# whoiszzj/APD-MVS

Measured on AMD Instinct MI355X. Metric: Mpix*iterations/sec (PatchMatch sweep), higher is better.
Workload: dtype f32

## Files before the change

apd-mvs_amd/csrc/apd_kernels_k67w.hip:

```cpp
#include "apd_device.h"
#include "apd_sweep.h"
#include "apd_window.h"


namespace apd {

constexpr int kWinH = APD_WIN_H;

template <bool kQuad>
__device__ __forceinline__ SrcWindow stage_window(const FrameArgs &fa, const ViewConst &vc, uint32_t *win, bool alive, int px, int py,
                                                  const float4 plane, bool trusted, bool enabled)
{
    if (!enabled) {
        SrcWindow none;
        none.valid = 0;
        none.wx0 = none.wy0 = none.addr0 = 0;
        none.lo_x = none.lo_y = 3.0e38f;
        none.hi_x = none.hi_y = -3.0e38f;
        return none;
    }
    float cx = 0.0f, cy = 0.0f;
    bool ok = false;
    if (alive) {
        float qx, qy, qz;
        plane_q(plane, qx, qy, qz);
        const Homography H = make_homography(fa, vc, qx, qy, qz);
        correspond(H, (float)px, (float)py, cx, cy);
        ok = cx >= 0.0f && cx < vc.wf && cy >= 0.0f && cy < vc.hf;
    }
    if (__builtin_amdgcn_ballot_w64(ok && trusted) != 0) {
        ok = ok && trusted;
    }
    return stage_window_around<kQuad, kWinH>(fa, vc, win, ok, cx, cy);
}

constexpr float kTrustedCost = 0.5f;
constexpr int kWinFromIter = 1;

template <int NMAX, bool kQuad, bool kTiled, bool kApprox>
__global__ __launch_bounds__(256, kQuad ? APD_K67W_WAVES : APD_K67W_WAVES_F32) void k67w_update_strong(FrameArgs fa, int colour, int iter)
{
    __shared__ float tile[kLdsH * kLdsPitch];
    __shared__ uint32_t windows[4][window_dwords(kWinH)];
    __shared__ uint16_t refine_items[4][5 * 64];
    __shared__ float refine_cost[4][5][64];
    const TilePixel t = checkerboard_pixel(fa, colour);
    for (int idx = threadIdx.x; idx < kLdsW * kLdsH; idx += 256) {
        const int r = idx / kLdsW, c = idx - r * kLdsW;
        tile[r * kLdsPitch + c] = fetch_texel(fa.ref_img, fa.W, fa.H, t.tx0 + c - kHalo, t.ty0 + r - kHalo);
    }
    __syncthreads();
    uint32_t *win = windows[threadIdx.x >> 6];
    const int px = t.px, py = t.py;
    const int center = py * fa.W + px;
    const bool alive = checkerboard_active(fa, t) && fa.weak_info[center] != APD_WEAK && !masked_out(fa, center);
    if (__builtin_amdgcn_ballot_w64(alive) == 0) {
        return;
    }
    const RefPatchLds<kLdsPitch> rp = ref_patch_from_lds<kLdsPitch>(&tile[t.ly * kLdsPitch + t.lx]);

    const int nsrc = fa.num_src;
    Rng rng = Rng{0, 0, 0, 0, 0, 0};
    float cost_array[9][NMAX];
    int positions[8];
    unsigned flags = 0;
    ViewWeights<NMAX> vw;
    vw.clear();
    float weight_norm = 0.0f;
    uint32_t sel = 0;
    float4 plane_now = make_float4(0.0f, 0.0f, 1.0f, 1.0f);
    float depth_now = 0.0f, cost_now = 0.0f, cost_committed = 0.0f;
    float ref_w[5];
    float4 ref_normals[5];
    float tc[5] = {0.0f, 0.0f, 0.0f, 0.0f, 0.0f};

    const bool use_windows = !(fa.state == APD_FIRST_INIT && iter < kWinFromIter);
    bool trusted = false;
    if (alive) {
        plane_now = fa.planes[center];
        trusted = fa.costs[center] < kTrustedCost;
#pragma unroll 1
        for (int h = 0; h < 8; ++h) {
            int pos = 0;
            if (arm_candidate(fa, px, py, h, pos)) {
                flags |= 1u << h;
            }
            positions[h] = pos;
        }
    }

#pragma unroll 1
    for (int v = 0; v < nsrc; ++v) {
        const ViewConst &vc = view_const(fa, v);
        const SrcWindow w = stage_window<kQuad>(fa, vc, win, alive, px, py, plane_now, trusted, use_windows);
        if (alive) {
#pragma unroll 1
            for (int h = 0; h < 9; ++h) {
                if (h < 8 && !(flags & (1u << h))) {
                    cost_array[h][v] = (h == 0 && v == 0) ? 2.0f : 0.0f;
                    continue;
                }
                const float4 pl = (h < 8) ? fa.planes[positions[h]] : plane_now;
                float qx, qy, qz;
                plane_q(pl, qx, qy, qz);
                cost_array[h][v] = ncc_fixed_windowed<kQuad, kWinW, kTiled, kApprox>(fa, vc, w, rp, px, py, qx, qy, qz);
            }
        }
    }

    if (alive) {
        float priors[NMAX];
        for (int j = 0; j < NMAX; ++j) {
            priors[j] = 0.0f;
        }
        const int nb_pos[4] = {center - fa.W, center + fa.W, center - 1, center + 1};
        for (int i = 0; i < 4; ++i) {
            if (flags & (1u << (2 * i))) {
                const uint32_t sv = fa.selected_views[nb_pos[i]];
                for (int j = 0; j < nsrc; ++j) {
                    priors[j] += bit_test(sv, (unsigned)j) == 1 ? 0.9f : 0.1f;
                }
            }
        }
        rng = rng_load(fa.rng, center);
        select_views<NMAX>(fa, iter, cost_array, priors, rng, vw, sel, weight_norm);
        vw.store(fa, center);
        float final_costs[8];
        for (int i = 0; i < 8; ++i) {
            float f = 0.0f;
            for (int j = 0; j < nsrc; ++j) {
                const uint32_t wj = vw.get(j);
                if (wj > 0) {
                    f += (float)wj * cost_array[i][j];
                }
            }
            final_costs[i] = f / weight_norm;
        }
        int best = 0;
        float best_c = final_costs[0];
        for (int i = 1; i < 8; ++i) {
            if (final_costs[i] <= best_c) {
                best_c = final_costs[i];
                best = i;
            }
        }
        cost_now = 0.0f;
        for (int i = 0; i < nsrc; ++i) {
            cost_now += (float)vw.get(i) * cost_array[8][i];
        }
        cost_now /= weight_norm;
        cost_committed = cost_now;
        depth_now = depth_from_plane(fa, plane_now, px, py);
        if (flags & (1u << best)) {
            const float4 cand = fa.planes[positions[best]];
            const float d = depth_from_plane(fa, cand, px, py);
            if (d >= fa.depth_min && d <= fa.depth_max && final_costs[best] < cost_now) {
                depth_now = d;
                plane_now = cand;
                cost_now = final_costs[best];
                fa.selected_views[center] = sel;
            }
        }
        float ref_depths[5];
        trusted = cost_now < kTrustedCost;
        make_refinement_set(fa, px, py, rng, plane_now, depth_now, ref_depths, ref_normals);
        rng_store(fa.rng, center, rng);
#pragma unroll
        for (int k = 0; k < 5; ++k) {
            ref_w[k] = distance_to_origin(fa, px, py, ref_depths[k], ref_normals[k].x, ref_normals[k].y, ref_normals[k].z);
        }
    }

    const float lost = refinement_lost_bound(fa, cost_now, weight_norm);
    const int lane = threadIdx.x & 63, wave_id = threadIdx.x >> 6;
    uint16_t *items = refine_items[wave_id];
    float(*costs_out)[64] = refine_cost[wave_id];
    const int wave_lx0 = (wave_id % kWavesX) * kWaveW, wave_ly0 = (wave_id / kWavesX) * kWaveH;
#pragma unroll 1
    for (int v = 0; v < nsrc; ++v) {
        const uint32_t wv = alive ? vw.get(v) : 0u;
        unsigned open = 0;
        if (wv > 0) {
#pragma unroll
            for (int k = 0; k < 5; ++k) {
                open |= (tc[k] >= lost) ? 0u : (1u << k);
            }
        }
        constexpr int kOrder[5] = {1, 3, 4, 0, 2};
        int off[6];
        off[0] = 0;
#pragma unroll
        for (int j = 0; j < 5; ++j) {
            const int k = kOrder[j];
            const unsigned long long m = __builtin_amdgcn_ballot_w64((open >> k) & 1u);
            if ((open >> k) & 1u) {
                const int rank = (int)__builtin_amdgcn_mbcnt_hi((unsigned)(m >> 32), __builtin_amdgcn_mbcnt_lo((unsigned)m, 0u));
                items[off[j] + rank] = (uint16_t)((k << 6) | lane);
            }
            off[j + 1] = off[j] + __builtin_popcountll(m);
        }
        const int total = off[5];
        if (total == 0) {
            continue;
        }
        __builtin_amdgcn_fence(__ATOMIC_RELEASE, "wavefront");
        __builtin_amdgcn_wave_barrier();
        const ViewConst &vc = view_const(fa, v);
        const SrcWindow w = stage_window<kQuad>(fa, vc, win, alive, px, py, plane_now, trusted, use_windows);
#pragma unroll 1
        for (int first = 0; first < total; first += 64) {
            const int idx = first + lane;
            const bool valid = idx < total;
            const unsigned item = valid ? (unsigned)items[idx] : 0u;
            const int owner = (int)(item & 63u), hyp = (int)(item >> 6);
            const int last = min(total, first + 64) - 1;
            int j_lo = 0, j_hi = 0;
#pragma unroll
            for (int j = 1; j < 5; ++j) {
                j_lo += off[j] <= first ? 1 : 0;
                j_hi += off[j] <= last ? 1 : 0;
            }
            float4 pl = make_float4(0.0f, 0.0f, 1.0f, 1.0f);
#pragma unroll 1
            for (int j = j_lo; j <= j_hi; ++j) {
                const int k = (0x20431 >> (4 * j)) & 7;
                const float nx = __shfl(ref_normals[k].x, owner), ny = __shfl(ref_normals[k].y, owner), nz = __shfl(ref_normals[k].z, owner);
                const float nw = __shfl(ref_w[k], owner);
                if (hyp == k) {
                    pl = make_float4(nx, ny, nz, nw);
                }
            }
            RefPatchLds<kLdsPitch> orp;
            orp.mean = __shfl(rp.mean, owner);
            orp.var = __shfl(rp.var, owner);
            const int oly = wave_ly0 + owner / kWaveLanesX;
            const int olx = wave_lx0 + 2 * (owner % kWaveLanesX) + ((oly + colour) & 1);
            orp.base = &tile[oly * kLdsPitch + olx];
            if (valid) {
                float qx, qy, qz;
                plane_q(pl, qx, qy, qz);
                costs_out[hyp][owner] = ncc_fixed_windowed<kQuad, kWinW, kTiled, kApprox>(fa, vc, w, orp, t.tx0 + olx, t.ty0 + oly, qx, qy, qz);
            }
        }
        __builtin_amdgcn_fence(__ATOMIC_RELEASE, "wavefront");
        __builtin_amdgcn_wave_barrier();
#pragma unroll
        for (int k = 0; k < 5; ++k) {
            if ((open >> k) & 1u) {
                tc[k] += (float)wv * costs_out[k][lane];
            }
        }
        __builtin_amdgcn_fence(__ATOMIC_RELEASE, "wavefront");
        __builtin_amdgcn_wave_barrier();
    }

    if (!alive) {
        return;
    }
#pragma unroll 1
    for (int k = 0; k < 5; ++k) {
        float4 pl = ref_normals[k];
        pl.w = ref_w[k];
        const float c = tc[k] / weight_norm;
        const float d = depth_from_plane(fa, pl, px, py);
        if (d >= fa.depth_min && d <= fa.depth_max && c < cost_now) {
            depth_now = d;
            plane_now = pl;
            cost_now = c;
        }
    }
    if (fa.state == APD_REFINE_INIT) {
        if ((double)cost_now < (double)cost_committed - 0.1) {
            fa.costs[center] = cost_now;
            fa.planes[center] = plane_now;
        } else {
            fa.costs[center] = cost_committed;
        }
    } else {
        fa.costs[center] = cost_now;
        fa.planes[center] = plane_now;
    }
}


template <bool kQuad, bool kTiled, bool kApprox>
static void launch_k67w_n(const FrameArgs &fa, int tiles, int colour, int iter, hipStream_t s)
{
    with_view_capacity(fa.num_src, [&](auto nmax) {
        hipLaunchKernelGGL((k67w_update_strong<decltype(nmax)::value, kQuad, kTiled, kApprox>), dim3(tiles), dim3(256), 0, s, fa, colour, iter);
    });
}

template <bool kQuad, bool kTiled>
static void launch_k67w(const FrameArgs &fa, int tiles, int colour, int iter, hipStream_t s)
{
    if (fa.approx_rcp) {
        launch_k67w_n<kQuad, kTiled, true>(fa, tiles, colour, iter, s);
    } else {
        launch_k67w_n<kQuad, kTiled, false>(fa, tiles, colour, iter, s);
    }
}

hipError_t launch_k67_windowed(const FrameArgs &fa, int colour, int iter, hipStream_t s)
{
    const int tiles = ((fa.W + kTileW - 1) / kTileW) * ((fa.H + kTileH - 1) / kTileH);
    if (fa.use_quads) {
        const int mode = fa.tiled_mode;
        const bool windows_off = fa.state == APD_FIRST_INIT && iter < kWinFromIter;
        if (fa.have_tiled && (mode == 2 || (mode == 1 && windows_off))) {
            launch_k67w<true, true>(fa, tiles, colour, iter, s);
        } else {
            launch_k67w<true, false>(fa, tiles, colour, iter, s);
        }
    } else {
        launch_k67w<false, false>(fa, tiles, colour, iter, s);
    }
    return hipGetLastError();
}

}


APD_WIN_STATS_ACCESSOR(apd_debug_win_stats)
```

apd-mvs_amd/csrc/apd_tuning.h:

```cpp
#pragma once

#ifndef APD_ROW_PREFETCH
#define APD_ROW_PREFETCH 1
#endif

#ifndef APD_CB_ROWS
#define APD_CB_ROWS 4
#endif
#ifndef APD_FF_ROWS
#define APD_FF_ROWS 8
#endif

#ifndef APD_WIN_H
#define APD_WIN_H (kWaveH + 16)
#endif
#ifndef APD_K67W_WAVES
#define APD_K67W_WAVES 4
#endif
#ifndef APD_K67W_WAVES_F32
#define APD_K67W_WAVES_F32 3
#endif

#ifndef APD_FW_TILE_PITCH
#define APD_FW_TILE_PITCH (kFwLds + 1)
#endif
#ifndef APD_K1415_WIN_PITCH
#define APD_K1415_WIN_PITCH 72
#endif
#ifndef APD_K14_WIN_H
#define APD_K14_WIN_H 32
#endif
#ifndef APD_K14_PAIRS_FROM_N
#define APD_K14_PAIRS_FROM_N 10
#endif
#ifndef APD_K14_PAIRS_FROM_N_PHOTO
#define APD_K14_PAIRS_FROM_N_PHOTO 8
#endif
#ifndef APD_K14_PAIRS_FROM_N_GEOM
#define APD_K14_PAIRS_FROM_N_GEOM 2
#endif
#ifndef APD_K14_PAIRS_MIN_SAVE
#define APD_K14_PAIRS_MIN_SAVE 2
#endif
#ifndef APD_K14_CHUNK
#define APD_K14_CHUNK 8
#endif
#ifndef APD_K14W_WAVES
#define APD_K14W_WAVES 4
#endif
#ifndef APD_K1415W_WAVES_F32
#define APD_K1415W_WAVES_F32 3
#endif

#ifndef APD_WEAK_SUPER_SHIFT
#define APD_WEAK_SUPER_SHIFT 4
#endif
#ifndef APD_K910_WIN_H
#define APD_K910_WIN_H 28
#endif
#ifndef APD_K910_WAVES
#define APD_K910_WAVES 2
#endif
```

apd-mvs_amd/csrc/apd_window.h:

```cpp
#pragma once

#include "apd_device.h"


namespace apd {

constexpr int kWinW = 64;
constexpr int window_dwords(int winh, int pitch = kWinW) { return pitch * (winh + 1); }
static_assert(kQuadShift == 2, "the window is staged from dword fetches of the quad image");

template <bool kQuad> struct WinEntry;
template <> struct WinEntry<true> {
    typedef uint32_t type;
};
template <> struct WinEntry<false> {
    typedef pair_t type;
};
constexpr int kWinEntryShift = 2;

typedef __attribute__((address_space(3))) uint32_t *lds_u32_ptr;

__device__ __forceinline__ int lds_address(uint32_t *p)
{
#if defined(__HIP_DEVICE_COMPILE__)
    return (int)(uintptr_t)(lds_u32_ptr)p;
#else
    return 0;
#endif
}

template <typename E>
struct WinTaps {
    E top, bot;
};

template <typename E, int kPitch>
__device__ __forceinline__ WinTaps<E> lds_read_pair(int addr)
{
    WinTaps<E> t;
#if defined(__HIP_DEVICE_COMPILE__)
    typedef __attribute__((address_space(3))) E *lds_ptr;
    const lds_ptr p = (lds_ptr)(uintptr_t)(uint32_t)addr;
    t.top = p[0];
    t.bot = p[kPitch];
#else
    t.top = t.bot = E();
#endif
    return t;
}

template <int kPitch>
__device__ __forceinline__ WinTaps<pair_t> lds_read_texels(int addr)
{
    WinTaps<pair_t> t;
#if defined(__HIP_DEVICE_COMPILE__)
    typedef __attribute__((address_space(3))) float *lds_ptr;
    const lds_ptr p = (lds_ptr)(uintptr_t)(uint32_t)addr;
    t.top.x = p[0];
    t.top.y = p[1];
    t.bot.x = p[kPitch];
    t.bot.y = p[kPitch + 1];
#else
    t.top = t.bot = pair_t();
#endif
    return t;
}


struct SrcWindow {
    int valid;
    int wx0, wy0;
    float lo_x, hi_x, lo_y, hi_y;
    int addr0;
};

__device__ __forceinline__ float wave_min(float v)
{
#pragma unroll
    for (int m = 32; m >= 1; m >>= 1) {
        v = fminf(v, __shfl_xor(v, m));
    }
    return v;
}

__device__ __forceinline__ float wave_max(float v)
{
#pragma unroll
    for (int m = 32; m >= 1; m >>= 1) {
        v = fmaxf(v, __shfl_xor(v, m));
    }
    return v;
}

template <bool kQuad, int WINH, int kPitch = kWinW>
__device__ __forceinline__ SrcWindow stage_window_around(const FrameArgs &fa, const ViewConst &vc, uint32_t *win, bool ok, float cx, float cy)
{
    constexpr int kWinRows = WINH + 1;
    SrcWindow w;
    const float big = 3.0e38f;
    const float x_lo = wave_min(ok ? cx : big), x_hi = wave_max(ok ? cx : -big);
    const float y_lo = wave_min(ok ? cy : big), y_hi = wave_max(ok ? cy : -big);
    if (!(x_lo <= x_hi)) {
        w.valid = 0;
        w.wx0 = w.wy0 = w.addr0 = 0;
        w.lo_x = w.lo_y = big;
        w.hi_x = w.hi_y = -big;
        return w;
    }
    const int wx0 = __builtin_amdgcn_readfirstlane((int)floorf(0.5f * (x_lo + x_hi)) - kWinW / 2);
    const int wy0 = __builtin_amdgcn_readfirstlane((int)floorf(0.5f * (y_lo + y_hi)) - WINH / 2);
    const int lane = threadIdx.x & 63;
    const int col = med3_i32(wx0 + lane, -1, fa.W - 1) + 1;
    if constexpr (kQuad) {
        const global_quad_ptr srcq = (global_quad_ptr)vc.quad;
        const unsigned rpitch = quad_row_pitch_bytes(fa.W);
        constexpr int kLoads = (kWinRows + 1) / 2;
        uint32_t tmp[kLoads];
#pragma unroll
        for (int k = 0; k < kLoads; ++k) {
            const int gy = min(max(wy0 + 2 * k, -1), fa.H - 1);
            tmp[k] = quad_fetch(srcq, (unsigned)(gy + 1) * rpitch + ((unsigned)col << kRowEntryShift));
        }
#pragma unroll
        for (int k = 0; k < kLoads; ++k) {
            float t0, t1, x0, x1;
            asm("v_cvt_f32_ubyte0 %0, %1" : "=v"(t0) : "v"(tmp[k]));
            asm("v_cvt_f32_ubyte1 %0, %1" : "=v"(t1) : "v"(tmp[k]));
            asm("v_cvt_f32_ubyte2 %0, %1" : "=v"(x0) : "v"(tmp[k]));
            asm("v_cvt_f32_ubyte3 %0, %1" : "=v"(x1) : "v"(tmp[k]));
            win[(2 * k) * kPitch + lane] = __builtin_bit_cast(uint32_t, __builtin_amdgcn_cvt_pkrtz(t0, x0 - t0));
            if (2 * k + 1 < kWinRows) {
                win[(2 * k + 1) * kPitch + lane] = __builtin_bit_cast(uint32_t, __builtin_amdgcn_cvt_pkrtz(t1, x1 - t1));
            }
        }
    } else {
        typedef const __attribute__((address_space(1))) float *global_float_ptr;
        const global_float_ptr img = (global_float_ptr)vc.img;
        float *winf = reinterpret_cast<float *>(win);
        const int cx = med3_i32(wx0 + lane, 0, fa.W - 1);
        float tmp[kWinRows];
#pragma unroll
        for (int k = 0; k < kWinRows; ++k) {
            const int gy = min(max(wy0 + k, 0), fa.H - 1);
            tmp[k] = img[(unsigned)(gy * fa.W + cx)];
        }
#pragma unroll
        for (int k = 0; k < kWinRows; ++k) {
            winf[k * kPitch + lane] = tmp[k];
        }
    }
    __builtin_amdgcn_fence(__ATOMIC_RELEASE, "wavefront");
    __builtin_amdgcn_wave_barrier();
    if ((threadIdx.x & 63) == 0) {
        APD_WIN_COUNT(5, 1);
    }
    w.valid = 1;
    w.wx0 = wx0;
    w.wy0 = wy0;
    w.lo_x = (float)max(wx0 + 1, 0);
    w.hi_x = (float)(wx0 + kWinW - (kQuad ? 1 : 2));
    w.lo_y = (float)max(wy0 + 1, 0);
    w.hi_y = (float)(wy0 + WINH - 1);
    w.addr0 = __builtin_amdgcn_readfirstlane(lds_address(win) - (wy0 * kPitch + wx0) * (1 << kWinEntryShift));
    return w;
}

template <int kShift, int kPitch>
__device__ __forceinline__ int win_byte_address(int qx, int qy, int addr0)
{
    int row, off;
    asm("v_mad_i32_i24 %0, %1, %2, %3" : "=v"(row) : "v"(qy), "v"(kPitch << kShift), "v"(addr0));
    asm("v_lshl_add_u32 %0, %1, %3, %2" : "=v"(off) : "v"(qx), "v"(row), "n"(kShift));
    return off;
}

template <bool kQuad, int kPitch, bool kApprox = false, bool kEnds = false>
__device__ __forceinline__ void win_row_issue(const Homography &H, float bx, float by, float bz, const float (&yf)[kPatchN], int addr0,
                                              float (&a)[kPatchN], float (&b)[kPatchN],
                                              WinTaps<typename WinEntry<kQuad>::type> (&t)[kPatchN], float Xa = 0.0f, float Ya = 0.0f,
                                              float Xb = 0.0f, float Yb = 0.0f)
{
    constexpr int j0 = kEnds ? 1 : 0, j1 = kEnds ? kPatchN - 1 : kPatchN;
    float z[kPatchN], X[kPatchN], Y[kPatchN], r[kPatchN];
#pragma unroll
    for (int j = j0; j < j1; ++j) {
        z[j] = fmaf(H.h[7], yf[j], bz);
        X[j] = fmaf(H.h[1], yf[j], bx);
        Y[j] = fmaf(H.h[4], yf[j], by);
    }
    APD_STAGE();
#pragma unroll
    for (int j = j0; j < j1; ++j) {
        r[j] = __builtin_amdgcn_rcpf(z[j]);
    }
    APD_STAGE();
    if constexpr (!kApprox) {
#pragma unroll
        for (int j = j0; j < j1; ++j) {
            z[j] = fmaf(-z[j], r[j], 1.0f);
        }
        APD_STAGE();
#pragma unroll
        for (int j = j0; j < j1; ++j) {
            r[j] = fmaf(z[j], r[j], r[j]);
        }
        APD_STAGE();
    }
#pragma unroll
    for (int j = j0; j < j1; ++j) {
        X[j] *= r[j];
        Y[j] *= r[j];
    }
    if constexpr (kEnds) {
        X[0] = Xa;
        Y[0] = Ya;
        X[kPatchN - 1] = Xb;
        Y[kPatchN - 1] = Yb;
    }
    APD_STAGE();
    constexpr float kEntryBytes = (float)(1 << kWinEntryShift), kPitchBytes = (float)(kPitch << kWinEntryShift);
    const float addr0f = (float)addr0 + 8388608.0f;
    float fx[kPatchN], fy[kPatchN];
#pragma unroll
    for (int j = 0; j < kPatchN; ++j) {
        a[j] = __builtin_amdgcn_fractf(X[j]);
        b[j] = __builtin_amdgcn_fractf(Y[j]);
    }
    APD_STAGE();
#pragma unroll
    for (int j = 0; j < kPatchN; ++j) {
        fx[j] = X[j] - a[j];
        fy[j] = Y[j] - b[j];
    }
    APD_STAGE();
#pragma unroll
    for (int j = 0; j < kPatchN; ++j) {
        fx[j] = fmaf(fx[j], kEntryBytes, addr0f);
    }
    APD_STAGE();
#pragma unroll
    for (int j = 0; j < kPatchN; ++j) {
        fx[j] = fmaf(fy[j], kPitchBytes, fx[j]);
    }
    APD_STAGE();
    int addr[kPatchN];
#pragma unroll
    for (int j = 0; j < kPatchN; ++j) {
        addr[j] = (int)(__float_as_uint(fx[j]) & 0x007FFFFFu);
    }
    APD_STAGE();
#pragma unroll
    for (int j = 0; j < kPatchN; ++j) {
        if constexpr (kQuad) {
            t[j] = lds_read_pair<uint32_t, kPitch>(addr[j]);
        } else {
            t[j] = lds_read_texels<kPitch>(addr[j]);
        }
    }
}

template <bool kQuad>
__device__ __forceinline__ void win_row_lerp(const WinTaps<typename WinEntry<kQuad>::type> (&t)[kPatchN], const float (&a)[kPatchN],
                                             const float (&b)[kPatchN], float (&v)[kPatchN])
{
    float top[kPatchN], bot[kPatchN];
#pragma unroll
    for (int j = 0; j < kPatchN; ++j) {
        if constexpr (kQuad) {
            top[j] = lerp_f16_pair(a[j], t[j].top);
            bot[j] = lerp_f16_pair(a[j], t[j].bot);
        } else {
            top[j] = fmaf(a[j], t[j].top.y - t[j].top.x, t[j].top.x);
            bot[j] = fmaf(a[j], t[j].bot.y - t[j].bot.x, t[j].bot.x);
        }
    }
    APD_STAGE();
#pragma unroll
    for (int j = 0; j < kPatchN; ++j) {
        bot[j] -= top[j];
    }
    APD_STAGE();
#pragma unroll
    for (int j = 0; j < kPatchN; ++j) {
        v[j] = fmaf(b[j], bot[j], top[j]);
    }
}

__device__ __forceinline__ float opaque_f32(float v)
{
    asm volatile("" : "+v"(v));
    return v;
}

template <bool kQuad, int kPitch, bool kApprox, bool kLocal = false, typename Ref>
__device__ __forceinline__ void ncc_window_moments(const Ref &rp, const Homography &H, int px, int py, int addr0, float &sum_s,
                                                   float &sum_ss, float &sum_rs, const float (&cX)[4], const float (&cY)[4])
{
    float yf[kPatchN];
    float x_first = 0.0f;
    if constexpr (kLocal) {
        x_first = opaque_f32((float)(px - kPatchRadius));
        const float y_first = opaque_f32((float)(py - kPatchRadius));
#pragma unroll
        for (int j = 0; j < kPatchN; ++j) {
            yf[j] = y_first + (float)(kPatchStep * j);
        }
    } else {
#pragma unroll
        for (int j = 0; j < kPatchN; ++j) {
            yf[j] = (float)(py + kPatchStep * j - kPatchRadius);
        }
    }
    sum_s = 0.0f;
    sum_ss = 0.0f;
    sum_rs = 0.0f;
    __builtin_amdgcn_s_setprio(1);
    __builtin_amdgcn_s_waitcnt(0xC07F);
    float a[2][kPatchN], b[2][kPatchN];
    WinTaps<typename WinEntry<kQuad>::type> t[2][kPatchN];
    {
        const float xf = kLocal ? x_first : (float)(px - kPatchRadius);
        win_row_issue<kQuad, kPitch, kApprox, true>(H, fmaf(H.h[0], xf, H.h[2]), fmaf(H.h[3], xf, H.h[5]), fmaf(H.h[6], xf, H.h[8]), yf,
                                                      addr0, a[0], b[0], t[0], cX[0], cY[0], cX[1], cY[1]);
    }
#pragma unroll
    for (int i = 0; i < kPatchN; ++i) {
        float v[kPatchN];
        float ref[kPatchN];
#pragma unroll
        for (int j = 0; j < kPatchN; ++j) {
            ref[j] = rp.at(i, j);
        }
        APD_STAGE();
        if (i + 2 < kPatchN) {
            const float xf = kLocal ? x_first + (float)(kPatchStep * (i + 1)) : (float)(px + kPatchStep * (i + 1) - kPatchRadius);
            win_row_issue<kQuad, kPitch, kApprox>(H, fmaf(H.h[0], xf, H.h[2]), fmaf(H.h[3], xf, H.h[5]), fmaf(H.h[6], xf, H.h[8]), yf,
                                                  addr0, a[(i + 1) & 1], b[(i + 1) & 1], t[(i + 1) & 1]);
        } else if (i + 1 < kPatchN) {
            const float xf = kLocal ? x_first + (float)(kPatchStep * (i + 1)) : (float)(px + kPatchStep * (i + 1) - kPatchRadius);
            win_row_issue<kQuad, kPitch, kApprox, true>(H, fmaf(H.h[0], xf, H.h[2]), fmaf(H.h[3], xf, H.h[5]), fmaf(H.h[6], xf, H.h[8]), yf,
                                                          addr0, a[(i + 1) & 1], b[(i + 1) & 1], t[(i + 1) & 1], cX[2], cY[2], cX[3], cY[3]);
        }
        APD_STAGE();
        win_row_lerp<kQuad>(t[i & 1], a[i & 1], b[i & 1], v);
        float row_s = 0.0f, row_ss = 0.0f, row_rs = 0.0f;
#pragma unroll
        for (int j = 0; j < kPatchN; ++j) {
            row_s += v[j];
            row_ss = fmaf(v[j], v[j], row_ss);
            row_rs = fmaf(ref[j], v[j], row_rs);
        }
        sum_s += row_s;
        sum_ss += row_ss;
        sum_rs += row_rs;
    }
    __builtin_amdgcn_s_setprio(0);
}

template <bool kApprox = false>
__device__ __forceinline__ void corner_position(const Homography &H, float xf, float yf, float &X, float &Y)
{
    const float z = fmaf(H.h[7], yf, fmaf(H.h[6], xf, H.h[8]));
    const float r = kApprox ? __builtin_amdgcn_rcpf(z) : recip_fast(z);
    X = fmaf(H.h[1], yf, fmaf(H.h[0], xf, H.h[2])) * r;
    Y = fmaf(H.h[4], yf, fmaf(H.h[3], xf, H.h[5])) * r;
}

template <bool kQuad, int kPitch = kWinW, bool kTiled = false, bool kApprox = false, bool kLocal = false, typename Ref>
__device__ __forceinline__ float ncc_fixed_windowed(const FrameArgs &fa, const ViewConst &vc, const SrcWindow &w, const Ref &rp, int px,
                                                    int py, float qx, float qy, float qz)
{
    const Homography H = make_homography(fa, vc, qx, qy, qz);
    float cx, cy;
    correspond(H, (float)px, (float)py, cx, cy);
    if (cx >= vc.wf || cx < 0.0f || cy >= vc.hf || cy < 0.0f) {
        return 2.0f;
    }
    const float kMinVar = 1e-5f;
    if (rp.var < kMinVar) {
        return 2.0f;
    }
    const float x0 = (float)(px - kPatchRadius), x1 = (float)(px + kPatchRadius);
    const float y0 = (float)(py - kPatchRadius), y1 = (float)(py + kPatchRadius);
    const bool fast_recip = denominators_fast(H, x0, x1, y0, y1);
    bool in_window = false;
    float cX[4], cY[4];
    if (fast_recip && w.valid) {
        corner_position<kApprox>(H, x0, y0, cX[0], cY[0]);
        corner_position<kApprox>(H, x0, y1, cX[1], cY[1]);
        corner_position<kApprox>(H, x1, y0, cX[2], cY[2]);
        corner_position<kApprox>(H, x1, y1, cX[3], cY[3]);
        const float xl = fminf(fminf(cX[0], cX[1]), fminf(cX[2], cX[3])), xh = fmaxf(fmaxf(cX[0], cX[1]), fmaxf(cX[2], cX[3]));
        const float yl = fminf(fminf(cY[0], cY[1]), fminf(cY[2], cY[3])), yh = fmaxf(fmaxf(cY[0], cY[1]), fmaxf(cY[2], cY[3]));
        in_window = xl >= w.lo_x && xh < w.hi_x && yl >= w.lo_y && yh < w.hi_y;
    }
    APD_LAB_NCC_STATS(in_window, fast_recip);
    in_window = in_window && __builtin_amdgcn_ballot_w64(!in_window) == 0;
    const bool fast_body = __builtin_amdgcn_ballot_w64(!fast_recip) == 0;
    float sum_s, sum_ss, sum_rs;
    if (in_window) {
        ncc_window_moments<kQuad, kPitch, kApprox, kLocal>(rp, H, px, py, w.addr0, sum_s, sum_ss, sum_rs, cX, cY);
    } else if constexpr (kApprox) {
        ncc_fixed_moments<kQuad, kRecipApprox, kTiled, Ref>(fa, vc, rp, H, px, py, sum_s, sum_ss, sum_rs);
    } else if (__builtin_expect(fast_body, 1)) {
        ncc_fixed_moments<kQuad, kRecipExact, kTiled, Ref>(fa, vc, rp, H, px, py, sum_s, sum_ss, sum_rs);
    } else {
        ncc_fixed_moments_ieee<kQuad, kTiled, Ref>(fa, vc, rp, H, px, py, sum_s, sum_ss, sum_rs);
    }
    const float inv_w = 1.0f / 36.0f;
    sum_s *= inv_w;
    sum_ss *= inv_w;
    sum_rs *= inv_w;
    const float var_s = fmaf(-sum_s, sum_s, sum_ss);
    if (var_s < kMinVar) {
        return 2.0f;
    }
    const float covar = fmaf(-rp.mean, sum_s, sum_rs);
    return ncc_cost_from_moments(rp.var, var_s, covar);
}

template <bool kQuad, int kPitch = kWinW, bool kTiled = false, bool kApprox = false, typename Ref>
__device__ __forceinline__ float ncc_fixed_windowed_from_h(const FrameArgs &fa, const ViewConst &vc, const SrcWindow &w, const Ref &rp,
                                                           const Homography &H, int px, int py)
{
    const float kMinVar = 1e-5f;
    if (rp.var < kMinVar) {
        return 2.0f;
    }
    const float x0 = (float)(px - kPatchRadius), x1 = (float)(px + kPatchRadius);
    const float y0 = (float)(py - kPatchRadius), y1 = (float)(py + kPatchRadius);
    const bool fast_recip = denominators_fast(H, x0, x1, y0, y1);
    bool in_window = false;
    float cX[4], cY[4];
    if (fast_recip && w.valid) {
        corner_position<kApprox>(H, x0, y0, cX[0], cY[0]);
        corner_position<kApprox>(H, x0, y1, cX[1], cY[1]);
        corner_position<kApprox>(H, x1, y0, cX[2], cY[2]);
        corner_position<kApprox>(H, x1, y1, cX[3], cY[3]);
        const float xl = fminf(fminf(cX[0], cX[1]), fminf(cX[2], cX[3])), xh = fmaxf(fmaxf(cX[0], cX[1]), fmaxf(cX[2], cX[3]));
        const float yl = fminf(fminf(cY[0], cY[1]), fminf(cY[2], cY[3])), yh = fmaxf(fmaxf(cY[0], cY[1]), fmaxf(cY[2], cY[3]));
        in_window = xl >= w.lo_x && xh < w.hi_x && yl >= w.lo_y && yh < w.hi_y;
    }
    APD_LAB_NCC_STATS(in_window, fast_recip);
    const bool fast_body = __builtin_amdgcn_ballot_w64(!fast_recip) == 0;
    float sum_s, sum_ss, sum_rs;
    if (in_window) {
        ncc_window_moments<kQuad, kPitch, kApprox>(rp, H, px, py, w.addr0, sum_s, sum_ss, sum_rs, cX, cY);
    } else if constexpr (kApprox) {
        ncc_fixed_moments<kQuad, kRecipApprox, kTiled, Ref>(fa, vc, rp, H, px, py, sum_s, sum_ss, sum_rs);
    } else if (__builtin_expect(fast_body, 1)) {
        ncc_fixed_moments<kQuad, kRecipExact, kTiled, Ref>(fa, vc, rp, H, px, py, sum_s, sum_ss, sum_rs);
    } else {
        ncc_fixed_moments_ieee<kQuad, kTiled, Ref>(fa, vc, rp, H, px, py, sum_s, sum_ss, sum_rs);
    }
    const float inv_w = 1.0f / 36.0f;
    sum_s *= inv_w;
    sum_ss *= inv_w;
    sum_rs *= inv_w;
    const float var_s = fmaf(-sum_s, sum_s, sum_ss);
    if (var_s < kMinVar) {
        return 2.0f;
    }
    const float covar = fmaf(-rp.mean, sum_s, sum_rs);
    return ncc_cost_from_moments(rp.var, var_s, covar);
}

}
```

Before: 471.8.

## Share one source-image LDS window across the whole workgroup instead of per wave

Replaces the four per-wave LDS windows with a single workgroup-wide window sized to the tile height. Each wave reduces its projected-coordinate bounding box with packed u16 min/max, the boxes are merged through LDS, and all four waves cooperatively load the window rows. This cuts LDS footprint and duplicate global fetches of overlapping rows. In exchange it adds two __syncthreads per staging call and forces all waves to stage in lockstep, even waves with no refine work. It also risks more out-of-window misses when the waves' projections diverge.

```diff
diff --git a/apd-mvs_amd/csrc/apd_kernels_k67w.hip b/apd-mvs_amd/csrc/apd_kernels_k67w.hip
--- a/apd-mvs_amd/csrc/apd_kernels_k67w.hip
+++ b/apd-mvs_amd/csrc/apd_kernels_k67w.hip
@@ -5,11 +5,11 @@
 
 namespace apd {
 
-constexpr int kWinH = APD_WIN_H;
+constexpr int kWinH = APD_K67_WG_WIN_H;
 
 template <bool kQuad>
-__device__ __forceinline__ SrcWindow stage_window(const FrameArgs &fa, const ViewConst &vc, uint32_t *win, bool alive, int px, int py,
-                                                  const float4 plane, bool trusted, bool enabled)
+__device__ __forceinline__ SrcWindow stage_window(const FrameArgs &fa, const ViewConst &vc, uint32_t *win, uint32_t *box, bool alive, int px,
+                                                  int py, const float4 plane, bool trusted, bool enabled, bool need)
 {
     if (!enabled) {
         SrcWindow none;
@@ -28,10 +28,7 @@
         correspond(H, (float)px, (float)py, cx, cy);
         ok = cx >= 0.0f && cx < vc.wf && cy >= 0.0f && cy < vc.hf;
     }
-    if (__builtin_amdgcn_ballot_w64(ok && trusted) != 0) {
-        ok = ok && trusted;
-    }
-    return stage_window_around<kQuad, kWinH>(fa, vc, win, ok, cx, cy);
+    return stage_window_around_wg<kQuad, kWinH>(fa, vc, win, box, ok, trusted, need, cx, cy);
 }
 
 constexpr float kTrustedCost = 0.5f;
@@ -41,7 +38,9 @@
 __global__ __launch_bounds__(256, kQuad ? APD_K67W_WAVES : APD_K67W_WAVES_F32) void k67w_update_strong(FrameArgs fa, int colour, int iter)
 {
     __shared__ float tile[kLdsH * kLdsPitch];
-    __shared__ uint32_t windows[4][window_dwords(kWinH)];
+    __shared__ uint32_t win[window_dwords(kWinH)];
+    __shared__ uint32_t box[kWgBoxDwords];
+    __shared__ uint32_t wave_live[4];
     __shared__ uint16_t refine_items[4][5 * 64];
     __shared__ float refine_cost[4][5][64];
     const TilePixel t = checkerboard_pixel(fa, colour);
@@ -49,12 +48,15 @@
         const int r = idx / kLdsW, c = idx - r * kLdsW;
         tile[r * kLdsPitch + c] = fetch_texel(fa.ref_img, fa.W, fa.H, t.tx0 + c - kHalo, t.ty0 + r - kHalo);
     }
-    __syncthreads();
-    uint32_t *win = windows[threadIdx.x >> 6];
     const int px = t.px, py = t.py;
     const int center = py * fa.W + px;
     const bool alive = checkerboard_active(fa, t) && fa.weak_info[center] != APD_WEAK && !masked_out(fa, center);
-    if (__builtin_amdgcn_ballot_w64(alive) == 0) {
+    const bool wave_alive = __builtin_amdgcn_ballot_w64(alive) != 0;
+    if ((threadIdx.x & 63) == 0) {
+        wave_live[threadIdx.x >> 6] = wave_alive ? 1u : 0u;
+    }
+    __syncthreads();
+    if ((wave_live[0] | wave_live[1] | wave_live[2] | wave_live[3]) == 0) {
         return;
     }
     const RefPatchLds<kLdsPitch> rp = ref_patch_from_lds<kLdsPitch>(&tile[t.ly * kLdsPitch + t.lx]);
@@ -92,7 +94,7 @@
 #pragma unroll 1
     for (int v = 0; v < nsrc; ++v) {
         const ViewConst &vc = view_const(fa, v);
-        const SrcWindow w = stage_window<kQuad>(fa, vc, win, alive, px, py, plane_now, trusted, use_windows);
+        const SrcWindow w = stage_window<kQuad>(fa, vc, win, box, alive, px, py, plane_now, trusted, use_windows, true);
         if (alive) {
 #pragma unroll 1
             for (int h = 0; h < 9; ++h) {
@@ -200,13 +202,13 @@
             off[j + 1] = off[j] + __builtin_popcountll(m);
         }
         const int total = off[5];
+        const ViewConst &vc = view_const(fa, v);
+        const SrcWindow w = stage_window<kQuad>(fa, vc, win, box, alive, px, py, plane_now, trusted, use_windows, total != 0);
         if (total == 0) {
             continue;
         }
         __builtin_amdgcn_fence(__ATOMIC_RELEASE, "wavefront");
         __builtin_amdgcn_wave_barrier();
-        const ViewConst &vc = view_const(fa, v);
-        const SrcWindow w = stage_window<kQuad>(fa, vc, win, alive, px, py, plane_now, trusted, use_windows);
 #pragma unroll 1
         for (int first = 0; first < total; first += 64) {
             const int idx = first + lane;
diff --git a/apd-mvs_amd/csrc/apd_tuning.h b/apd-mvs_amd/csrc/apd_tuning.h
--- a/apd-mvs_amd/csrc/apd_tuning.h
+++ b/apd-mvs_amd/csrc/apd_tuning.h
@@ -11,8 +11,8 @@
 #define APD_FF_ROWS 8
 #endif
 
-#ifndef APD_WIN_H
-#define APD_WIN_H (kWaveH + 16)
+#ifndef APD_K67_WG_WIN_H
+#define APD_K67_WG_WIN_H (kTileH + 16)
 #endif
 #ifndef APD_K67W_WAVES
 #define APD_K67W_WAVES 4
diff --git a/apd-mvs_amd/csrc/apd_window.h b/apd-mvs_amd/csrc/apd_window.h
--- a/apd-mvs_amd/csrc/apd_window.h
+++ b/apd-mvs_amd/csrc/apd_window.h
@@ -153,6 +153,138 @@
     __builtin_amdgcn_wave_barrier();
     if ((threadIdx.x & 63) == 0) {
         APD_WIN_COUNT(5, 1);
+    }
+    w.valid = 1;
+    w.wx0 = wx0;
+    w.wy0 = wy0;
+    w.lo_x = (float)max(wx0 + 1, 0);
+    w.hi_x = (float)(wx0 + kWinW - (kQuad ? 1 : 2));
+    w.lo_y = (float)max(wy0 + 1, 0);
+    w.hi_y = (float)(wy0 + WINH - 1);
+    w.addr0 = __builtin_amdgcn_readfirstlane(lds_address(win) - (wy0 * kPitch + wx0) * (1 << kWinEntryShift));
+    return w;
+}
+
+typedef unsigned short u16x2 __attribute__((ext_vector_type(2)));
+
+__device__ __forceinline__ uint32_t pk_min_u16(uint32_t a, uint32_t b)
+{
+    return __builtin_bit_cast(uint32_t, __builtin_elementwise_min(__builtin_bit_cast(u16x2, a), __builtin_bit_cast(u16x2, b)));
+}
+
+__device__ __forceinline__ uint32_t pk_max_u16(uint32_t a, uint32_t b)
+{
+    return __builtin_bit_cast(uint32_t, __builtin_elementwise_max(__builtin_bit_cast(u16x2, a), __builtin_bit_cast(u16x2, b)));
+}
+
+constexpr int kWgBoxDwords = 16;
+
+template <bool kQuad, int WINH>
+__device__ __forceinline__ SrcWindow stage_window_around_wg(const FrameArgs &fa, const ViewConst &vc, uint32_t *win, uint32_t *box, bool ok,
+                                                            bool preferred, bool need, float cx, float cy)
+{
+    constexpr int kPitch = kWinW;
+    constexpr int kWinRows = WINH + 1;
+    const int lane = threadIdx.x & 63, wave = threadIdx.x >> 6;
+    const bool wave_preferred = __builtin_amdgcn_ballot_w64(ok && preferred) != 0;
+    if (wave_preferred) {
+        ok = ok && preferred;
+    }
+    const uint32_t p = ok ? ((uint32_t)(int)cx | ((uint32_t)(int)cy << 16)) : 0u;
+    uint32_t lo = ok ? p : 0xFFFFFFFFu, hi = p;
+#pragma unroll
+    for (int m = 32; m >= 1; m >>= 1) {
+        lo = pk_min_u16(lo, (uint32_t)__shfl_xor((int)lo, m));
+        hi = pk_max_u16(hi, (uint32_t)__shfl_xor((int)hi, m));
+    }
+    if (lane == 0) {
+        box[4 * wave + 0] = lo;
+        box[4 * wave + 1] = hi;
+        box[4 * wave + 2] = (wave_preferred ? 2u : 0u) | (need ? 1u : 0u);
+    }
+    __syncthreads();
+    uint32_t any = 0;
+#pragma unroll
+    for (int k = 0; k < 4; ++k) {
+        any |= box[4 * k + 2];
+    }
+    lo = 0xFFFFFFFFu;
+    hi = 0u;
+#pragma unroll
+    for (int k = 0; k < 4; ++k) {
+        if (!(any & 2u) || (box[4 * k + 2] & 2u)) {
+            lo = pk_min_u16(lo, box[4 * k + 0]);
+            hi = pk_max_u16(hi, box[4 * k + 1]);
+        }
+    }
+    lo = (uint32_t)__builtin_amdgcn_readfirstlane((int)lo);
+    hi = (uint32_t)__builtin_amdgcn_readfirstlane((int)hi);
+    any = (uint32_t)__builtin_amdgcn_readfirstlane((int)any);
+    const int x_lo = (int)(lo & 0xFFFFu), y_lo = (int)(lo >> 16), x_hi = (int)(hi & 0xFFFFu), y_hi = (int)(hi >> 16);
+    const bool valid = (any & 1u) != 0 && x_lo <= x_hi;
+    const int wx0 = ((x_lo + x_hi + 1) >> 1) - kWinW / 2;
+    const int wy0 = ((y_lo + y_hi + 1) >> 1) - WINH / 2;
+    if (valid) {
+        if constexpr (kQuad) {
+            const int col = med3_i32(wx0 + lane, -1, fa.W - 1) + 1;
+            const global_quad_ptr srcq = (global_quad_ptr)vc.quad;
+            const unsigned rpitch = quad_row_pitch_bytes(fa.W);
+            constexpr int kLoads = (kWinRows + 1) / 2, kPerWave = (kLoads + 3) / 4;
+            uint32_t tmp[kPerWave];
+#pragma unroll
+            for (int i = 0; i < kPerWave; ++i) {
+                const int k = min(wave + 4 * i, kLoads - 1);
+                const int gy = min(max(wy0 + 2 * k, -1), fa.H - 1);
+                tmp[i] = quad_fetch(srcq, (unsigned)(gy + 1) * rpitch + ((unsigned)col << kRowEntryShift));
+            }
+#pragma unroll
+            for (int i = 0; i < kPerWave; ++i) {
+                const int k = wave + 4 * i;
+                if (k < kLoads) {
+                    float t0, t1, x0, x1;
+                    asm("v_cvt_f32_ubyte0 %0, %1" : "=v"(t0) : "v"(tmp[i]));
+                    asm("v_cvt_f32_ubyte1 %0, %1" : "=v"(t1) : "v"(tmp[i]));
+                    asm("v_cvt_f32_ubyte2 %0, %1" : "=v"(x0) : "v"(tmp[i]));
+                    asm("v_cvt_f32_ubyte3 %0, %1" : "=v"(x1) : "v"(tmp[i]));
+                    win[(2 * k) * kPitch + lane] = __builtin_bit_cast(uint32_t, __builtin_amdgcn_cvt_pkrtz(t0, x0 - t0));
+                    if (2 * k + 1 < kWinRows) {
+                        win[(2 * k + 1) * kPitch + lane] = __builtin_bit_cast(uint32_t, __builtin_amdgcn_cvt_pkrtz(t1, x1 - t1));
+                    }
+                }
+            }
+        } else {
+            typedef const __attribute__((address_space(1))) float *global_float_ptr;
+            const global_float_ptr img = (global_float_ptr)vc.img;
+            float *winf = reinterpret_cast<float *>(win);
+            const int tx = med3_i32(wx0 + lane, 0, fa.W - 1);
+            constexpr int kPerWave = (kWinRows + 3) / 4;
+            float tmp[kPerWave];
+#pragma unroll
+            for (int i = 0; i < kPerWave; ++i) {
+                const int k = min(wave + 4 * i, kWinRows - 1);
+                const int gy = min(max(wy0 + k, 0), fa.H - 1);
+                tmp[i] = img[(unsigned)(gy * fa.W + tx)];
+            }
+#pragma unroll
+            for (int i = 0; i < kPerWave; ++i) {
+                const int k = wave + 4 * i;
+                if (k < kWinRows) {
+                    winf[k * kPitch + lane] = tmp[i];
+                }
+            }
+        }
+        if (threadIdx.x == 0) {
+            APD_WIN_COUNT(5, 1);
+        }
+    }
+    __syncthreads();
+    SrcWindow w;
+    if (!valid) {
+        w.valid = 0;
+        w.wx0 = w.wy0 = w.addr0 = 0;
+        w.lo_x = w.lo_y = 3.0e38f;
+        w.hi_x = w.hi_y = -3.0e38f;
+        return w;
     }
     w.valid = 1;
     w.wx0 = wx0;
```

Result: slower. 447.3 (-5.2%).
